# isabella232/Garfield

Hardware: AMD Instinct MI355X
Metric: img/sec ResNet-50 f=2 Multi-Krum (higher is better)
Workload: dtype bf16; 1 GPU; model=resnet50 (torchvision architecture, 10 classes, 23528522 params), global_batch=2000, parallelism=dp1 (robust DP, 8 logical workers/GPU, n=8), gar=krum, f=2, batch_per_worker=250, exchange_dtype=bf16, hip_graphs=True, worker_batching=True, lp_weights=True, optimizer=SGD lr=0.01 momentum=0.9 wd=5e-4 (fused into the GAR combine kernel)

## Files before the change

garfield_amd/csrc/bindings.cpp:

```cpp
#include <map>
#include <mutex>
#include <torch/extension.h>
#include <c10/hip/HIPGuard.h>
#include <c10/hip/HIPStream.h>

#include <cstdint>
#include <cstdlib>
#include <string>
#include <vector>

#include "bn_gpu.hpp"
#include "conv_f32.hpp"
#include "gar_common.hpp"
#include "gar_cpu.hpp"
#include "gar_gpu.hpp"
#include "loss_gpu.hpp"
#include "mailbox.hpp"
#include "threadpool.hpp"

namespace py = pybind11;
using garfield::RowTable;

namespace {

// ... 1399 lines not shown
  bool bf16 = false;
  int64_t ss = 0, gs = 0;
  if (out.scalar_type() == at::kFloat) {
    TORCH_CHECK(out.is_contiguous() && out.dim() == 4 && out.size(0) == splits && out.size(1) == groups &&
                    out.size(2) == cout && out.size(3) == K,
                "gpu_iwgrad: an fp32 out must be contiguous [splits, groups, Cout, K]");
    ss = groups * cout * K;
    gs = cout * K;
  } else {
    TORCH_CHECK(out.scalar_type() == at::kBFloat16 && splits == 1 && out.dim() == 3 && out.size(0) == groups &&
                    out.size(1) == cout && out.size(2) == K && out.stride(2) == 1 && out.stride(1) == K &&
                    out.stride(0) >= cout * K,
                "gpu_iwgrad: a bf16 out must be a [groups, Cout, K] view with contiguous rows (splits == 1)");
    bf16 = true;
    gs = out.stride(0);
  }
  const float* psc = opt_vec(pro_scale, groups * g.C, x.device(), "pro_scale");
  const float* psh = opt_vec(pro_shift, groups * g.C, x.device(), "pro_shift");
  TORCH_CHECK((psc == nullptr) == (psh == nullptr), "gpu_iwgrad: pass both pro_scale and pro_shift or neither");
  c10::hip::HIPGuard guard(x.device().index());
  if (psc) {
    TORCH_CHECK(kh == 1 && kw == 1 && sh == 1 && sw == 1 && ph == 0 && pw == 0,
                "gpu_iwgrad: the BatchNorm prologue takes 1x1 stride-1 unpadded convolutions only");
    garfield::gpu::iwgrad_nhwc(u16(x), u16(dy), g, static_cast<int>(cout), static_cast<int>(groups), M / groups,
                               static_cast<int>(splits), out.data_ptr(), bf16, ss, gs, stream_of(x.device()), psc, psh);
    return;
  }
  if (garfield::gpu::wgrad3x3_nhwc(u16(x), u16(dy), g, static_cast<int>(cout), static_cast<int>(groups),
                                         M / groups, static_cast<int>(splits), out.data_ptr(), bf16, ss, gs,
                                         stream_of(x.device())))
    return;
  garfield::gpu::iwgrad_nhwc(u16(x), u16(dy), g, static_cast<int>(cout), static_cast<int>(groups), M / groups,
                             static_cast<int>(splits), out.data_ptr(), bf16, ss, gs, stream_of(x.device()));
}

bool g_wgrad3x3_fits(int64_t n, int64_t h, int64_t w, int64_t c, int64_t cout, int64_t groups) {
  garfield::gpu::Im2col g{static_cast<int>(n), static_cast<int>(h), static_cast<int>(w), static_cast<int>(c), 3, 3,
                          1, 1, 1, 1, 1, 1, static_cast<int>(h), static_cast<int>(w), 0};
  if (groups < 1 || n % groups) return false;
  return garfield::gpu::wgrad3x3_fits(g, static_cast<int>(cout), n / groups * h * w);
}

garfield::gpu::Im2col pool_geometry(const at::Tensor& x, const at::Tensor& y, const at::Tensor& idx, int64_t k,
                                    int64_t s, int64_t p) {
  auto g = conv_geometry(x, k, k, s, s, p, p, 1, 1, true);
  TORCH_CHECK(g.C % 8 == 0 && reinterpret_cast<uintptr_t>(x.data_ptr()) % 16 == 0,
              "garfield maxpool: channels must be a multiple of 8 and x 16-byte aligned");
  TORCH_CHECK(y.device() == x.device() && y.scalar_type() == x.scalar_type() && y.dim() == 4 && y.size(0) == g.N &&
                  y.size(1) == g.C && y.size(2) == g.Ho && y.size(3) == g.Wo &&
                  y.is_contiguous(at::MemoryFormat::ChannelsLast) && reinterpret_cast<uintptr_t>(y.data_ptr()) % 16 == 0,
              "garfield maxpool: y must be a channels_last [", g.N, ", ", g.C, ", ", g.Ho, ", ", g.Wo, "] tensor of x's dtype");
  TORCH_CHECK(idx.device() == x.device() && idx.scalar_type() == at::kByte && idx.numel() == y.numel() &&
                  idx.is_contiguous() && reinterpret_cast<uintptr_t>(idx.data_ptr()) % 8 == 0 && k * k <= 256,
              "garfield maxpool: idx must be a contiguous uint8 tensor of y's element count");
  return g;
}

void g_maxpool_fwd(const at::Tensor& x, int64_t k, int64_t s, int64_t p, const at::Tensor& y, const at::Tensor& idx) {
  auto g = pool_geometry(x, y, idx, k, s, p);
  c10::hip::HIPGuard guard(x.device().index());
  garfield::gpu::maxpool_fwd_nhwc(x.data_ptr(), g, y.data_ptr(), static_cast<uint8_t*>(idx.data_ptr()),
                                  stream_of(x.device()), dtype_code(x));
}

void g_maxpool_bwd(const at::Tensor& dy, const at::Tensor& idx, int64_t k, int64_t s, int64_t p, const at::Tensor& dx) {
  auto g = pool_geometry(dx, dy, idx, k, s, p);
// ... 582 lines not shown
  m.def("gpu_iconv", &g_iconv, "Implicit-GEMM NHWC convolution on MFMA: y = conv(x, w) (+ add); args (x, w, kh, kw, "
        "sh, sw, ph, pw, dh, dw, y, add=None, pm=0, transpose_w=False); x/y/add channels_last bf16, C % 32 == 0, "
        "Cout % 64 == 0; transpose_w: w is the forward weight [C, Cout, KH, KW] whose flipped transpose is applied "
        "(the data gradient of that convolution); add_mask [y.numel() / 8] uint8: add counts where its bit is set "
        "(halo-staged 3x3 kernel only, y a separate tensor). Returns False when nothing was launched (add_mask on a "
        "shape the halo kernel does not take)",
        py::arg("x"), py::arg("w"), py::arg("kh"), py::arg("kw"), py::arg("sh"), py::arg("sw"), py::arg("ph"),
        py::arg("pw"), py::arg("dh"), py::arg("dw"), py::arg("y"), py::arg("add") = py::none(), py::arg("pm") = 0,
        py::arg("transpose_w") = false, py::arg("stats") = py::none(), py::arg("rg") = 0,
        py::arg("add_mask") = py::none());
  m.def("conv3x3_stats_rows", [](int64_t n, int64_t h, int64_t w, int64_t c, int64_t cout) -> int64_t {
          return 16 * g_conv3x3_pick(n, h, w, c, cout);
        }, py::arg("n"), py::arg("h"), py::arg("w"), py::arg("c"), py::arg("cout"),
        "Rows per statistics tile of the halo-staged 3x3 kernel's BatchNorm-statistics epilogue (0: no fit); "
        "the stats buffer holds ceil(M / rows) * 6 * Cout floats (E = 1)");

  m.def("gpu_sc_expand", &g_sc_expand, py::arg("weights"), py::arg("hs"), py::arg("ws"), py::arg("bigs"),
        py::arg("bigTs"), "Per-step expansion of 3x3 weights for images of at most 2x2 pixels: Wbig[(p', co), (p, ci)] "
        "= W[co, h - h' + 1, w - w' + 1, ci] (0 off the kernel) and its transpose, every layer in one launch");
  m.def("gpu_sc_fold", &g_sc_fold, py::arg("slab"), py::arg("h"), py::arg("w"), py::arg("out"),
        "Fold a dense small-image weight gradient (fp32 [S, G, P*Cout, P*Cin]) onto the nine taps: out[g, co, "
        "(i, j, ci)] = Σ_s Σ over the pixel pairs of tap (i, j)");
  m.def("gpu_dgrad_s2", &g_dgrad_s2, "Data gradient of a stride-2 convolution on MFMA without a dcol matrix: dx = "
        "conv_transpose(dy, w) (+ add, in place of add when given; dx may be add); args (dy, w, kh, kw, ph, pw, dx, "
        "add=None, pm=0); w the channels_last forward weight [C, Cout, KH, KW]", py::arg("dy"), py::arg("w"),
        py::arg("kh"), py::arg("kw"), py::arg("ph"), py::arg("pw"), py::arg("dx"), py::arg("add") = py::none(),
        py::arg("pm") = 0);
  m.def("dgrad_s2_ok", &g_dgrad_s2_ok, py::arg("dy"), py::arg("dx"), py::arg("kh"), py::arg("kw"), py::arg("ph"),
        py::arg("pw"), "True when gpu_dgrad_s2 takes this geometry");
  m.def("conv3x3_pick", &g_conv3x3_pick, py::arg("n"), py::arg("h"), py::arg("w"), py::arg("c"), py::arg("cout"),
        "Pixel fragments per wave the halo-staged 3x3 kernel uses for this NHWC shape (0: it does not fit)");
  m.def("wgrad3x3_fits", &g_wgrad3x3_fits, py::arg("n"), py::arg("h"), py::arg("w"), py::arg("c"), py::arg("cout"),
        py::arg("groups"), "True when gpu_iwgrad of this 3x3 / stride-1 / pad-1 shape runs the halo-staged kernel");
  m.def("gpu_iwgrad", &g_iwgrad, "Per-worker implicit-GEMM weight gradient on MFMA: out[s, g] = Σ over pixel "
        "split s of worker g of dyᵀ · patches(x); args (x, dy, kh, kw, sh, sw, ph, pw, dh, dw, groups, out, splits, "
        "pro_scale=None, pro_shift=None); pro_*: [groups, C] BatchNorm prologue of x (1x1 only)",
        py::arg("x"), py::arg("dy"), py::arg("kh"), py::arg("kw"), py::arg("sh"), py::arg("sw"), py::arg("ph"),
        py::arg("pw"), py::arg("dh"), py::arg("dw"), py::arg("groups"), py::arg("out"), py::arg("splits"),
        py::arg("pro_scale") = py::none(), py::arg("pro_shift") = py::none());
  m.def("gpu_conv_f32", &g_conv_f32, py::arg("src"), py::arg("w"), py::arg("kh"), py::arg("kw"),
        py::arg("sh"), py::arg("sw"), py::arg("ph"), py::arg("pw"), py::arg("dh"), py::arg("dw"), py::arg("dgrad"),
        py::arg("out"), py::arg("add") = py::none(), py::arg("pm") = 0, py::arg("ksplit") = 0,
        "fp32 NHWC implicit-GEMM convolution (forward, or with dgrad the data gradient of a convolution of this "
        "geometry, any stride) on split-bf16 MFMA (three bf16 pieces per operand, the six products of order <= 2, "
        "fp32 accumulation); w: the weight's pieces [3, Co, K]; pm 0: automatic kernel choice (split-K included "
        "unless ksplit is given), ksplit > 1: that many k-splits summed by a second pass");
  m.def("conv_f32_supported", [](int64_t cs, int64_t co) {
    garfield::gpu::ConvF32Geo g{};
    g.Cs = static_cast<int>(cs);
    g.Co = static_cast<int>(co);
    return garfield::gpu::conv_f32_supported(g);
  }, py::arg("cs"), py::arg("co"));
  m.def("gpu_wgrad_f32", &g_wgrad_f32, py::arg("x"), py::arg("dy"), py::arg("kh"), py::arg("kw"), py::arg("sh"),
        py::arg("sw"), py::arg("ph"), py::arg("pw"), py::arg("dh"), py::arg("dw"), py::arg("groups"), py::arg("out"),
        py::arg("splits"), py::arg("variant") = 0,
        "Per-worker fp32 weight gradient on split-bf16 MFMA (variant: 0 auto, 1 / 2 the 128x128 tile double- / "
        "single-buffered, 3 the 64x64 tile)");
  m.def("gpu_wsplit_multi", &g_wsplit_multi, "Per-step weight split of many fp32 weights: W -> its three bf16 "
        "pieces (row pitch ld) and, optionally, the channel-transposed pieces of the data gradient");
  m.def("gpu_linear_f32_fwd", [](const at::Tensor& x, const at::Tensor& w, const c10::optional<at::Tensor>& b,
                                 const at::Tensor& y) {
    const auto dev = x.device();
    const int64_t R = x.size(0), F = x.size(1), O = w.size(0);
    check_f32_mat(x, dev, R, F, "x");
    check_f32_mat(w, dev, O, F, "w");
    check_f32_mat(y, dev, R, O, "y");
// ... 315 lines not shown
```

garfield_amd/csrc/bn_gpu.hpp:

```cpp
#pragma once
#include <hip/hip_runtime.h>
#include <cstdint>

namespace garfield {
namespace gpu {

constexpr int kBnMaxChunks = 64;

int64_t bn_part_floats(int64_t rg, int groups, int C);

struct RunJob {
  const float* mean;
  const float* istd;
  float* run_mean;
  float* run_var;
  int64_t rg;
  int C;
  int groups;
  float eps;
  float momentum;
};
constexpr int kRunJobs = 48;
struct RunJobs {
  RunJob j[kRunJobs];
// ... 71 lines not shown
int conv3x3_pick(const Im2col& g, int Cout);
struct ScExpandJob {
  const uint16_t* w;
  uint16_t* big;
  uint16_t* bigT;
  int cout, cin, H, W;
};
constexpr int kScMaxJobs = 32;
struct ScExpandJobs {
  ScExpandJob job[kScMaxJobs];
  int64_t start[kScMaxJobs + 1];
  int count;
};
void sc_expand(const ScExpandJobs& jobs, hipStream_t stream);
void sc_fold(const float* slab, int S, int G, int H, int W, int cout, int cin, void* out, bool out_bf16,
             int64_t gstride, hipStream_t stream);

bool dgrad_s2_ok(const Im2col& g, int Cout);
void dgrad_s2_nhwc(const uint16_t* dy, const uint16_t* w, const Im2col& g, int Cout, uint16_t* dx, const uint16_t* add,
                   int pm, hipStream_t stream);
bool conv3x3_nhwc(const uint16_t* x, const uint16_t* w, const Im2col& g, int Cout, uint16_t* y, const uint16_t* add,
                  int pmf, hipStream_t stream, float* stats = nullptr, int64_t rg = 0,
                  const uint8_t* add_mask = nullptr);
bool wgrad3x3_fits(const Im2col& g, int Cout, int64_t rg);
bool wgrad3x3_nhwc(const uint16_t* x, const uint16_t* dy, const Im2col& g, int Cout, int groups, int64_t rg,
                   int splits, void* out, bool out_bf16, int64_t split_stride, int64_t group_stride,
                   hipStream_t stream);
void maxpool_fwd_nhwc(const void* x, const Im2col& g, void* y, uint8_t* idx, hipStream_t stream, int dt = 1);
void maxpool_bwd_nhwc(const void* dy, const uint8_t* idx, const Im2col& g, void* dx, hipStream_t stream, int dt = 1);
int iwgrad_taps_per_block(int kw, int kh = 3, int C = 0, int Cout = 0);
void iwgrad_nhwc(const uint16_t* x, const uint16_t* dy, const Im2col& g, int Cout, int groups, int64_t rg,
                 int splits, void* out, bool out_bf16, int64_t split_stride, int64_t group_stride, hipStream_t stream,
                 const float* pro_scale = nullptr, const float* pro_shift = nullptr);
void col2im_nhwc(const uint16_t* dcol, const Im2col& g, uint16_t* dx, bool accumulate, hipStream_t stream);

}
}
```

garfield_amd/csrc/iconv_nhwc.hip:

```cpp
#include <cstdlib>

#include "bn_gpu.hpp"
#include "gar_device.hpp"

namespace garfield {
namespace gpu {
using namespace dev;
namespace {

constexpr int kWaves = 4;

__device__ __forceinline__ bf16x8 pro_frag(bf16x8 b, float sc, float sh) {
  const uint4 u = __builtin_bit_cast(uint4, b);
  const float x[8] = {__uint_as_float(u.x << 16), __uint_as_float(u.x & 0xffff0000u),
                      __uint_as_float(u.y << 16), __uint_as_float(u.y & 0xffff0000u),
                      __uint_as_float(u.z << 16), __uint_as_float(u.z & 0xffff0000u),
                      __uint_as_float(u.w << 16), __uint_as_float(u.w & 0xffff0000u)};
  float y[8];
#pragma unroll
  for (int i = 0; i < 8; ++i) y[i] = fmaxf(fmaf(x[i], sc, sh), 0.f);
  return __builtin_bit_cast(bf16x8, make_uint4(pack_bf16x2(y[0], y[1]), pack_bf16x2(y[2], y[3]),
                                               pack_bf16x2(y[4], y[5]), pack_bf16x2(y[6], y[7])));
}

template <int PM>
struct Frags {
  bf16x8 a[4];
  bf16x8 b[PM];
};

template <int PM, bool ADD>
__global__ __launch_bounds__(256) void k_iconv(const uint16_t* __restrict__ x, const uint16_t* __restrict__ w,
                                               Im2col g, int Cout, uint16_t* y, const uint16_t* add) {
// ... 822 lines not shown
#pragma unroll
    for (int j = 0; j < NT; ++j)
#pragma unroll
      for (int v = 0; v < 2; ++v) {
        bf16x8 bx =
            __builtin_bit_cast(bf16x8, __builtin_shufflevector(rb[j][2 * v], rb[j][2 * v + 1], 0, 1, 2, 3, 4, 5, 6, 7));
        if constexpr (PRO) bx = pro_frag(bx, psv[j][v], phv[j][v]);
#pragma unroll
        for (int u = 0; u < 2; ++u)
          acc[j][u][v] = __builtin_amdgcn_mfma_f32_16x16x32_bf16(a[u], bx, acc[j][u][v], 0, 0, 0);
      }
  }

#pragma unroll
  for (int j = 0; j < NT; ++j) {
    const int k0 = c0 + j * 64;
#pragma unroll
    for (int u = 0; u < 2; ++u)
#pragma unroll
      for (int v = 0; v < 2; ++v)
#pragma unroll
        for (int e = 0; e < 4; ++e) {
          const int co = co0 + (cf0 + u) * 16 + 4 * grp + e;
          const int64_t o = static_cast<int64_t>(sp) * split_stride + static_cast<int64_t>(gi) * group_stride +
                            static_cast<int64_t>(co) * K + k0 + (kf0 + v) * 16 + li;
          if constexpr (OUT_BF16) static_cast<uint16_t*>(out)[o] = f_to_bf16(acc[j][u][v][e]);
          else static_cast<float*>(out)[o] = acc[j][u][v][e];
        }
  }
}

constexpr int kW1Stage = 4 * 64 * 128;

template <bool OUT_BF16, bool PRO, int NS = 3>
__global__ __launch_bounds__(256) void k_iwgrad_1x1_wide(const uint16_t* __restrict__ x, const uint16_t* __restrict__ dy,
                                                         Im2col g, int Cout, int64_t rg, int64_t per_split, void* out,
                                                         int64_t split_stride, int64_t group_stride,
                                                         const float* __restrict__ psc, const float* __restrict__ psh) {
  constexpr int SUB = 64 * 128;
  extern __shared__ __attribute__((aligned(16))) char wlds[];
  const int lane = threadIdx.x & 63, wave = threadIdx.x >> 6;
  const int K = g.C;
  const int nq = g.C / 128;
  const int qb = blockIdx.x % nq, cb = blockIdx.x / nq;
  const int c0 = qb * 128, co0 = cb * 128;
  const int gi = blockIdx.y, sp = blockIdx.z;
  const int64_t mbeg = static_cast<int64_t>(gi) * rg + static_cast<int64_t>(sp) * per_split;
  int64_t mend = mbeg + per_split;
  if (mend > static_cast<int64_t>(gi + 1) * rg) mend = static_cast<int64_t>(gi + 1) * rg;
  const int steps = mend > mbeg ? static_cast<int>((mend - mbeg + 63) / 64) : 0;
  const FastDiv fWo = make_fastdiv(g.Wo), fHo = make_fastdiv(g.Ho);
  const bool ident = g.sh == 1 && g.sw == 1 && g.ph == 0 && g.pw == 0 && g.H == g.Ho && g.W == g.Wo;

  const int lchunk = lane & 7;
  const uint16_t* zsrc = reinterpret_cast<const uint16_t*>(g_iconv_zero) + lchunk * 8;
  const uint64_t az = reinterpret_cast<uint64_t>(zsrc);
  auto issue = [&](int s, int slot) {
    char* base = wlds + slot * kW1Stage;
#pragma unroll
    for (int hb = 0; hb < 2; ++hb) {
      const int row = 8 * (hb * 4 + wave) + (lane >> 3);
      const int lsw = lchunk ^ (2 * tr_g(row));
      const int m = static_cast<int>(mbeg) + s * 64 + row;
      const bool mv = m < static_cast<int>(mend);
      const int mm = mv ? m : 0;
      bool ok = mv;
      int64_t xo = mm;
      if (!ident) {
        uint32_t t, wo, n, ho;
        fdivmod(static_cast<uint32_t>(mm), fWo, t, wo);
        fdivmod(t, fHo, n, ho);
        const int hi = static_cast<int>(ho) * g.sh - g.ph, wi = static_cast<int>(wo) * g.sw - g.pw;
        ok = mv && hi >= 0 && hi < g.H && wi >= 0 && wi < g.W;
        xo = (static_cast<int64_t>(n) * g.H + (ok ? hi : 0)) * g.W + (ok ? wi : 0);
      }
      const uint16_t* dr = dy + static_cast<int64_t>(mm) * Cout + co0 + lsw * 8;
      const uint16_t* xr = x + xo * g.C + c0 + lsw * 8;
#pragma unroll
      for (int b = 0; b < 2; ++b) {
// ... 52 lines not shown
          "ds_read_b64_tr_b16 %4, %18\n\t"
          "ds_read_b64_tr_b16 %5, %18 offset:512\n\t"
          "ds_read_b64_tr_b16 %6, %19\n\t"
          "ds_read_b64_tr_b16 %7, %19 offset:512\n\t"
          "ds_read_b64_tr_b16 %8, %20\n\t"
          "ds_read_b64_tr_b16 %9, %20 offset:512\n\t"
          "ds_read_b64_tr_b16 %10, %21\n\t"
          "ds_read_b64_tr_b16 %11, %21 offset:512\n\t"
          "ds_read_b64_tr_b16 %12, %22\n\t"
          "ds_read_b64_tr_b16 %13, %22 offset:512\n\t"
          "ds_read_b64_tr_b16 %14, %23\n\t"
          "ds_read_b64_tr_b16 %15, %23 offset:512\n\t"
          "s_waitcnt lgkmcnt(0)"
          : "=&v"(ra[0]), "=&v"(ra[1]), "=&v"(ra[2]), "=&v"(ra[3]), "=&v"(ra[4]), "=&v"(ra[5]), "=&v"(ra[6]),
            "=&v"(ra[7]), "=&v"(rb[0]), "=&v"(rb[1]), "=&v"(rb[2]), "=&v"(rb[3]), "=&v"(rb[4]), "=&v"(rb[5]),
            "=&v"(rb[6]), "=&v"(rb[7])
          : "v"(b0 + offA[0]), "v"(b0 + offA[1]), "v"(b0 + offA[2]), "v"(b0 + offA[3]), "v"(b0 + offB[0]),
            "v"(b0 + offB[1]), "v"(b0 + offB[2]), "v"(b0 + offB[3])
          : "memory");
      bf16x8 a[4], b[4];
#pragma unroll
      for (int k = 0; k < 4; ++k) {
        a[k] = __builtin_bit_cast(bf16x8, __builtin_shufflevector(ra[2 * k], ra[2 * k + 1], 0, 1, 2, 3, 4, 5, 6, 7));
        b[k] = __builtin_bit_cast(bf16x8, __builtin_shufflevector(rb[2 * k], rb[2 * k + 1], 0, 1, 2, 3, 4, 5, 6, 7));
        if constexpr (PRO) b[k] = pro_frag(b[k], psv[k], phv[k]);
      }
#pragma unroll
      for (int u = 0; u < 4; ++u)
#pragma unroll
        for (int v = 0; v < 4; ++v) acc[u][v] = __builtin_amdgcn_mfma_f32_16x16x32_bf16(a[u], b[v], acc[u][v], 0, 0, 0);
    }
  }

#pragma unroll
  for (int u = 0; u < 4; ++u)
#pragma unroll
    for (int v = 0; v < 4; ++v)
#pragma unroll
      for (int e = 0; e < 4; ++e) {
        const int co = co0 + (4 * sa + u) * 16 + 4 * grp + e;
        const int k = c0 + (4 * sbk + v) * 16 + li;
        const int64_t o = static_cast<int64_t>(sp) * split_stride + static_cast<int64_t>(gi) * group_stride +
                          static_cast<int64_t>(co) * K + k;
        if constexpr (OUT_BF16) static_cast<uint16_t*>(out)[o] = f_to_bf16(acc[u][v][e]);
        else static_cast<float*>(out)[o] = acc[u][v][e];
      }
}

int iwgrad_taps_per_block(int kw, int kh, int C, int Cout) {
  if (kw == 1 && kh == 1) return C % 128 == 0 ? (Cout % 128 == 0 ? 4 : 2) : 1;
  return kw == 3 ? 3 : 1;
}

template <bool PRO>
void iwgrad_launch(const uint16_t* x, const uint16_t* dy, const Im2col& g, int Cout, int groups, int64_t rg,
                   int splits, void* out, bool out_bf16, int64_t split_stride, int64_t group_stride, hipStream_t stream,
                   const float* psc, const float* psh) {
  const int K = g.KH * g.KW * g.C;
  if (splits < 1) splits = 1;
  const int64_t per_split = (rg + splits - 1) / splits;
  const int tpb = iwgrad_taps_per_block(g.KW, g.KH, g.C, Cout);
  if (tpb == 4 && g.KW == 1) {
    static bool once = (hipFuncSetAttribute(reinterpret_cast<const void*>(&k_iwgrad_1x1_wide<true, PRO>),
                                            hipFuncAttributeMaxDynamicSharedMemorySize, 3 * kW1Stage),
                        hipFuncSetAttribute(reinterpret_cast<const void*>(&k_iwgrad_1x1_wide<false, PRO>),
                                            hipFuncAttributeMaxDynamicSharedMemorySize, 3 * kW1Stage),
                        hipFuncSetAttribute(reinterpret_cast<const void*>(&k_iwgrad_1x1_wide<true, PRO, 2>),
                                            hipFuncAttributeMaxDynamicSharedMemorySize, 2 * kW1Stage),
                        hipFuncSetAttribute(reinterpret_cast<const void*>(&k_iwgrad_1x1_wide<false, PRO, 2>),
                                            hipFuncAttributeMaxDynamicSharedMemorySize, 2 * kW1Stage),
                        true);
    (void)once;
    const dim3 grid((g.C / 128) * (Cout / 128), groups, splits);
    const bool ns2 = (per_split + 63) / 64 <= 4;
    if (out_bf16 && ns2)
      hipLaunchKernelGGL((k_iwgrad_1x1_wide<true, PRO, 2>), grid, dim3(256), 2 * kW1Stage, stream, x, dy, g, Cout, rg,
                         per_split, out, split_stride, group_stride, psc, psh);
    else if (out_bf16)
      hipLaunchKernelGGL((k_iwgrad_1x1_wide<true, PRO>), grid, dim3(256), 3 * kW1Stage, stream, x, dy, g, Cout, rg,
// ... 7 lines not shown
    return;
  }
  if (tpb == 2 && g.KW == 1) {
    const dim3 grid((g.C / 128) * (Cout / 64), groups, splits);
    if (out_bf16)
      hipLaunchKernelGGL((k_iwgrad_1x1<3, true, 2, PRO>), grid, dim3(256), 0, stream, x, dy, g, Cout, rg, per_split,
                         out, split_stride, group_stride, psc, psh);
    else
      hipLaunchKernelGGL((k_iwgrad_1x1<3, false, 2, PRO>), grid, dim3(256), 0, stream, x, dy, g, Cout, rg, per_split,
                         out, split_stride, group_stride, psc, psh);
    return;
  }
  if constexpr (!PRO) {
    if (tpb == 3) {
      const dim3 grid(g.KH * (g.C / 64) * (Cout / 64), groups, splits);
      if (out_bf16)
        hipLaunchKernelGGL((k_iwgrad_rows<3, true, 1>), grid, dim3(256), 0, stream, x, dy, g, Cout, rg, per_split, out,
                           split_stride, group_stride);
      else
        hipLaunchKernelGGL((k_iwgrad_rows<3, false, 1>), grid, dim3(256), 0, stream, x, dy, g, Cout, rg, per_split, out,
                           split_stride, group_stride);
      return;
    }
  }
  const dim3 grid((K / 64) * (Cout / 64), groups, splits);
  if (out_bf16)
    hipLaunchKernelGGL((k_iwgrad<3, true, PRO>), grid, dim3(256), 0, stream, x, dy, g, Cout, rg, per_split, out,
                       split_stride, group_stride, psc, psh);
  else
    hipLaunchKernelGGL((k_iwgrad<3, false, PRO>), grid, dim3(256), 0, stream, x, dy, g, Cout, rg, per_split, out,
                       split_stride, group_stride, psc, psh);
}

void iwgrad_nhwc(const uint16_t* x, const uint16_t* dy, const Im2col& g, int Cout, int groups, int64_t rg,
                 int splits, void* out, bool out_bf16, int64_t split_stride, int64_t group_stride, hipStream_t stream,
                 const float* pro_scale, const float* pro_shift) {
  if (pro_scale)
    iwgrad_launch<true>(x, dy, g, Cout, groups, rg, splits, out, out_bf16, split_stride, group_stride, stream,
                        pro_scale, pro_shift);
  else
    iwgrad_launch<false>(x, dy, g, Cout, groups, rg, splits, out, out_bf16, split_stride, group_stride, stream, nullptr,
                         nullptr);
}

}
}
```

garfield_amd/ops/grouped.py:

```python
from __future__ import annotations

import math

import torch
import torch.nn.functional as F

from garfield_amd import _native
from garfield_amd.ops import tuning
from garfield_amd.utils.flat import is_dense

ICONV = True
IWGRAD = True
IWGRAD_1X1 = True
STEM = True
_STEM_WG = 1024
XENT = True
GEMM_NT = True
GEMM_NT_DGRAD = True
CONV3X3 = True
BN_PROLOGUE = False
S2_DGRAD = True
_S2_CHOICE: dict = tuning.register("s2", {})
S2_FORCE = False
SMALL_CONV = True
LAZY_RES = True
FOLD_SHORTCUT_BN = True
BN_DUAL = True


def rows2d(t: torch.Tensor) -> torch.Tensor:
    if t.dim() == 2:
        return t
    if not t.is_contiguous(memory_format=torch.channels_last):
        raise ValueError("grouped layers need channels_last activations")
    return t.permute(0, 2, 3, 1).reshape(-1, t.shape[1])


def from_rows(t2: torch.Tensor, n: int, h: int, w: int) -> torch.Tensor:
    return t2.view(n, h, w, t2.shape[1]).permute(0, 3, 1, 2)


def _cl(t: torch.Tensor) -> torch.Tensor:
    return t.contiguous(memory_format=torch.channels_last) if t.dim() == 4 else t.contiguous()




class GradSink:

    def __init__(self, flat: torch.Tensor, row_stride: int, base: int, offsets: dict, groups: int):
        self.flat = flat
        self.row_stride = int(row_stride)
        self.base = int(base)
        self.offsets = offsets
        self.groups = int(groups)
        self._srcs: list = []
        self._offs: list = []
        self._split_parts: list = []
        self._split_outs: list = []
        self.defer_splits = True

    def offset(self, p: torch.Tensor) -> int:
        return self.offsets[id(p)]

    def row_offset(self, g: int, p: torch.Tensor) -> int:
        return self.base + g * self.row_stride + self.offsets[id(p)]

    def put(self, p: torch.Tensor, g: int, grad: torch.Tensor) -> None:
        if grad.numel() != p.numel():
            raise ValueError(f"gradient of {grad.numel()} elements for a parameter of {p.numel()}")
        self._srcs.append(grad)
        self._offs.append(self.row_offset(g, p))

    def rows_view(self, p: torch.Tensor, shape: tuple, dtype: torch.dtype) -> torch.Tensor | None:
        if self.flat.dtype != dtype:
            return None
        strides, acc = [], 1
        for d in reversed(shape):
            strides.append(acc)
            acc *= int(d)
        if acc != p.numel():
            raise ValueError(f"rows_view of {acc} elements for a parameter of {p.numel()}")
        return self.flat.as_strided((self.groups, *shape), (self.row_stride, *reversed(strides)),
                                    self.base + self.offsets[id(p)])

    def queue_split(self, part: torch.Tensor, out: torch.Tensor) -> None:
        if self.defer_splits and part.is_cuda:
            self._split_parts.append(part)
            self._split_outs.append(out)
        else:
            _native.native().gpu_split_reduce(part, out)

    def put_groups(self, p: torch.Tensor, grads) -> None:
        for g in range(self.groups):
            self.put(p, g, grads[g])

    def flush_splits(self) -> None:
        if self._split_parts:
            _native.native().gpu_split_reduce_multi(self._split_parts, self._split_outs)
            self._split_parts.clear()
            self._split_outs.clear()

    def flush(self) -> None:
        self.flush_splits()
        if not self._srcs:
            return
        if self.flat.is_cuda:
            srcs = [s if is_dense(s) else s.contiguous() for s in self._srcs]
            _native.native().gpu_flatten_cast_at(srcs, self._offs, self.flat)
        else:
            with torch.no_grad():
                for s, o in zip(self._srcs, self._offs):
                    v = _memory_order(s)
                    self.flat[o:o + v.numel()].copy_(v)
        self._srcs.clear()
        self._offs.clear()


def _memory_order(t: torch.Tensor) -> torch.Tensor:
    if t.is_contiguous():
        return t.reshape(-1)
    perm = sorted(range(t.dim()), key=lambda i: -t.stride(i))
    return t.permute(perm).reshape(-1)


class GradJoin:

    __slots__ = ("pending", "lazy")

    def __init__(self):
# ... 253 lines not shown
        else:
            dx2, dr2 = _bn_bwd_ref(x2, dy2, y2, st, ctx.has_res)
            dx = from_rows(dx2, n, h, w)
            dres = from_rows(dr2, n, h, w) if dr2 is not None else None
        if lazy is not None:
            if ctx.join is not None:
                ctx.join.park(lazy)
            else:
                ctx.res_link.pending = lazy
        elif dres is not None and ctx.join is not None:
            ctx.join.park(dres)
            dres = None
        return dx, None, None, dres, None, None, None, None, None, None


def grouped_bn(x, st: BNState, ws: Workspace, res=None, res_join: GradJoin | None = None,
               res_link: ResLink | None = None, out_link: ResLink | None = None, res_st: BNState | None = None):
    return _GroupedBN.apply(_cl(x), st.bn.weight, st.bn.bias, _cl(res) if res is not None else None, st, ws,
                            res_join, res_link, out_link, res_st)




class ConvSpec:
    def __init__(self, conv: torch.nn.Conv2d, sink: GradSink | None, groups: int):
        if conv.groups != 1 or conv.bias is not None:
            raise ValueError("grouped convolution supports groups=1 convolutions without bias")
        self.conv = conv
        self.sink = sink
        self.groups = groups
        self.kernel = tuple(conv.kernel_size)
        self.stride = tuple(conv.stride)
        self.padding = tuple(conv.padding)
        self.dilation = tuple(conv.dilation)
        self.gemm = (self.kernel == (1, 1) and self.stride == (1, 1) and self.padding == (0, 0)
                     and self.dilation == (1, 1))
        self.bn_next = None
        self.wpad = None
        self.wt = None
        self.dcol = False
        self.wd = None
        self.flip = False
        self.w3 = self.wt3 = None
        self.sc = None
        self.wbig = self.wbigT = None


def _gemm_nt_ok(a2: torch.Tensor, b2: torch.Tensor) -> bool:
    M, K = a2.shape
    N = b2.shape[0]
    return (a2.is_cuda and a2.dtype == torch.bfloat16 and b2.dtype == torch.bfloat16 and K % 64 == 0
            and N % 64 == 0 and b2.shape[1] == K and a2.is_contiguous() and b2.is_contiguous()
            and M * max(K, N) < 2 ** 31)


_GEMM_CFG: dict = tuning.register("gemm", {})


def _gemm_cfg(a2: torch.Tensor, b2: torch.Tensor, rg: int, add: torch.Tensor | None, pro=None) -> int:
    C_ = _native.native()
    M, K = a2.shape
    N = b2.shape[0]
    key = (M, N, K, rg, add is not None, pro is not None)
    cfg = _GEMM_CFG.get(key)
    if cfg is not None:
        return cfg
# ... 377 lines not shown
    while S < _IWGRAD_MAXS and tiles * S < _IWGRAD_WG and rows_per_worker // (2 * S) >= _IWGRAD_MINPIX:
        S *= 2
    return S


def _wgrad3x3_splits(rows_per_worker: int, blocks: int) -> int:
    tiles = -(-rows_per_worker // 128)
    S = 1
    while S < 64 and blocks * S < _WGRAD3_WG and tiles // (2 * S) >= _WGRAD3_MINTILES:
        S *= 2
    return S


_WGRAD3_WG = 512
_WGRAD3_MINTILES = 3


_IWGRAD_WG = 512
_IWGRAD_MINPIX = 512
_IWGRAD_MAXS = 64


def _iwgrad(x: torch.Tensor, dy: torch.Tensor, spec: "ConvSpec", G: int, K: int, pro=None) -> None:
    pkw = {} if pro is None else {"pro_scale": pro[0], "pro_shift": pro[1]}
    cout = dy.shape[1]
    rows = dy.shape[0] * dy.shape[2] * dy.shape[3] // G
    C_ = _native.native()
    if (CONV3X3 and spec.kernel == (3, 3) and spec.stride == (1, 1) and spec.padding == (1, 1)
            and spec.dilation == (1, 1) and C_.wgrad3x3_fits(x.shape[0], x.shape[2], x.shape[3], x.shape[1], cout, G)):
        S = _wgrad3x3_splits(rows, (x.shape[1] // 64) * (cout // 64) * G)
    else:
        S = _iwgrad_splits(rows, (K // 64) * (cout // 64) * G //
                          C_.iwgrad_taps_per_block(spec.kernel[1], spec.kernel[0], x.shape[1], cout))
    out = spec.sink.rows_view(spec.conv.weight, (cout, K), dy.dtype) if S == 1 else None
    if out is not None:
        C_.gpu_iwgrad(x, dy, *_geom(spec), G, out, 1, **pkw)
        return
    part = torch.empty((S, G, cout, K), dtype=torch.float32, device=dy.device)
    C_.gpu_iwgrad(x, dy, *_geom(spec), G, part, S, **pkw)
    rows = spec.sink.rows_view(spec.conv.weight, (cout, K), spec.sink.flat.dtype)
    if rows is not None:
        spec.sink.queue_split(part, rows)
    else:
        spec.sink.put_groups(spec.conv.weight, part.sum(0) if S > 1 else part[0])


def _stem_kind(w: torch.Tensor, spec: "ConvSpec") -> int | None:
    if spec.dilation != (1, 1):
        return None
    if tuple(w.shape) == (64, 3, 7, 7) and spec.stride == (2, 2) and spec.padding == (3, 3):
        return 0
    if tuple(w.shape) == (64, 3, 3, 3) and spec.stride == (1, 1) and spec.padding == (1, 1):
        return 1
    return None


def _stem_ok(x: torch.Tensor, w: torch.Tensor, spec: "ConvSpec") -> bool:
    kind = _stem_kind(w, spec)
    return (STEM and kind is not None and x.is_cuda and x.dtype == torch.bfloat16 and w.dtype == torch.bfloat16
            and _channels_last_weight(w) and x.is_contiguous(memory_format=torch.channels_last)
            and _native.native().stem_supported(x.shape[2], x.shape[3], kind))


def _stem_wgrad(x: torch.Tensor, dy: torch.Tensor, spec: "ConvSpec", G: int) -> None:
    per = x.shape[0] // G
    wg = _STEM_WG * (2 if dy.shape[2] * dy.shape[3] > 4096 else 1)
    S = max(1, min(per, -(-wg // G)))
    C_ = _native.native()
    kind = _stem_kind(spec.conv.weight, spec) or 0
    K = C_.stem_k(kind)
    part = torch.empty((S, G, 64, K), dtype=torch.float32, device=dy.device)
    C_.gpu_stem_wgrad(x, dy, G, part, kind)
    rows = spec.sink.rows_view(spec.conv.weight, (64, K), spec.sink.flat.dtype)
# ... 787 lines not shown
```

garfield_amd/parallel/grouped.py:

```python
from __future__ import annotations

import torch
import torch.nn as nn
import torch.nn.functional as F

from garfield_amd.models.resnet import BasicBlock, Bottleneck, ResNet
from garfield_amd.parallel.signals import DeviceSignal
from garfield_amd.ops.grouped import (BNState, ConvSpec, GradJoin, GradSink, LinearSpec, ResLink, Workspace,
                                      bn_conv_ok, global_avgpool, grouped_bn, grouped_bn_conv, grouped_conv,
                                      grouped_cross_entropy, grouped_linear, grouped_maxpool, refresh_dgrad_weights,
                                      refresh_f32_weights, refresh_sc_weights)
import garfield_amd.ops.grouped as _gops


def supports(model: nn.Module) -> bool:
    if not isinstance(model, ResNet):
        return False
    for m in model.modules():
        if isinstance(m, nn.BatchNorm2d):
            if m.num_features % 8 or m.momentum is None or not m.affine:
                return False
        elif isinstance(m, nn.Conv2d):
            if m.groups != 1 or m.bias is not None:
                return False
# ... 22 lines not shown
            kh, kw = mod.kernel_size
            if mod is not model.conv1 and kh * kw > 1 and tuple(mod.stride) != (1, 1):
                sizes.append(out.numel() // mod.out_channels * mod.in_channels * kh * kw)

    hooks = [m.register_forward_hook(hook) for m in model.modules()
             if isinstance(m, (nn.Conv2d, nn.BatchNorm2d, nn.MaxPool2d, nn.ReLU, nn.Linear, nn.AdaptiveAvgPool2d))]
    state = {n: torch.empty_like(t, device="meta") for n, t in [*model.named_parameters(), *model.named_buffers()]}
    try:
        with torch.no_grad():
            torch.func.functional_call(model, state, (torch.empty((rows, *sample_shape), device="meta"),))
    finally:
        for h in hooks:
            h.remove()
    _CAPACITY[key] = out = max(sizes)
    return out


def fits(model: ResNet, rows: int, sample_shape) -> bool:
    return largest_index(model, rows, sample_shape) <= INDEX_LIMIT


class GroupedResNet:

    def __init__(self, model: ResNet, groups: int, sink: GradSink, loss_fn=F.cross_entropy, marks=(),
                 offsets: dict | None = None, signals: bool = True):
        if not supports(model):
            raise ValueError("GroupedResNet supports the zoo's ResNet models only")
        self.model = model
        self.groups = int(groups)
        self.sink = sink
        self.loss_fn = loss_fn
        self.ws = Workspace()
        self.conv = {m: ConvSpec(m, sink, self.groups) for m in model.modules() if isinstance(m, nn.Conv2d)}
        self.fc = LinearSpec(model.fc, sink, self.groups)
        self.bn: dict = {}
        self._seed = None
        self.join_residuals = True
        self.marks = tuple(marks)
        self._offsets = offsets or {}
        self._events = None
        self._end = None
        if signals and self.marks and next(model.parameters()).is_cuda:
            dev = next(model.parameters()).device
            self._events = {name: DeviceSignal(dev) for name in self.marks}
            self._end = DeviceSignal(dev)

    def bucket_offsets(self) -> list:
        out = []
        for name in self.marks:
            layer = getattr(self.model, name)
            offs = [self._offsets[id(p)] for p in layer.parameters() if id(p) in self._offsets]
            if offs:
                out.append(min(offs))
        return out

    def mark_events(self):
        if self._events is None:
            return None
        return [self._events[name] for name in self.marks] + [self._end]

    def replayed(self) -> None:
        for sgn in self.mark_events() or ():
            sgn.replayed()


    def _state(self, bn: nn.BatchNorm2d, relu: bool) -> BNState:
# ... 155 lines not shown
```

Measured before the change: 380,000 img/s.

## Batch small 1x1 weight-gradient GEMMs into one multi-job kernel launch per stage

Adds a multi-job variant of the wide 1x1 weight-gradient kernel that takes up to 16 layer jobs in one grid, with blocks mapped to jobs through prefix offsets and jobs sorted by work. Small 1x1 wgrad calls (fewer than 512 workgroups, no BN prologue) are queued in the gradient sink and flushed per ResNet stage or before split reduction. The aim is to cut launch count and fill the GPU better when individual layers launch too few workgroups. It delays wgrad work and keeps activations alive until the flush, and it adds a per-block linear job search.

After: 388,600 img/s, median of 6. 1.02x the previous value.

```diff
diff --git a/garfield_amd/csrc/bindings.cpp b/garfield_amd/csrc/bindings.cpp
--- a/garfield_amd/csrc/bindings.cpp
+++ b/garfield_amd/csrc/bindings.cpp
@@ -1455,6 +1455,69 @@
     return;
   garfield::gpu::iwgrad_nhwc(u16(x), u16(dy), g, static_cast<int>(cout), static_cast<int>(groups), M / groups,
                              static_cast<int>(splits), out.data_ptr(), bf16, ss, gs, stream_of(x.device()));
+}
+
+void g_iwgrad_multi(const std::vector<at::Tensor>& xs, const std::vector<at::Tensor>& dys,
+                    const std::vector<std::vector<int64_t>>& geoms, int64_t groups, const std::vector<at::Tensor>& outs,
+                    const std::vector<int64_t>& splits) {
+  const size_t n = xs.size();
+  TORCH_CHECK(dys.size() == n && geoms.size() == n && outs.size() == n && splits.size() == n,
+              "gpu_iwgrad_multi: xs, dys, geoms, outs and splits must have one entry per job");
+  if (n == 0) return;
+  std::vector<garfield::gpu::WgJob> jobs;
+  jobs.reserve(n);
+  const at::Device dev = xs[0].device();
+  int64_t wgs = 0;
+  for (size_t i = 0; i < n; ++i) {
+    const at::Tensor &x = xs[i], &dy = dys[i], &out = outs[i];
+    const auto& q = geoms[i];
+    TORCH_CHECK(q.size() == 8, "gpu_iwgrad_multi: a geometry is (kh, kw, sh, sw, ph, pw, dh, dw)");
+    TORCH_CHECK(x.device() == dev, "gpu_iwgrad_multi: every job must be on one device");
+    auto g = conv_geometry(x, q[0], q[1], q[2], q[3], q[4], q[5], q[6], q[7]);
+    TORCH_CHECK(dy.is_cuda() && dy.device() == dev && dy.scalar_type() == at::kBFloat16 && dy.dim() == 4 &&
+                    dy.is_contiguous(at::MemoryFormat::ChannelsLast) && dy.size(0) == g.N && dy.size(2) == g.Ho &&
+                    dy.size(3) == g.Wo,
+                "gpu_iwgrad_multi: dy must be a channels_last bf16 [", g.N, ", Cout, ", g.Ho, ", ", g.Wo, "] tensor");
+    const int64_t cout = dy.size(1);
+    TORCH_CHECK(cout <= INT32_MAX && garfield::gpu::iwgrad_wide_ok(g, static_cast<int>(cout)),
+                "gpu_iwgrad_multi: takes 1x1 convolutions with input and output channels multiples of 128 only (got ",
+                g.KH, "x", g.KW, ", ", g.C, " -> ", cout, ")");
+    const int64_t M = static_cast<int64_t>(g.N) * g.Ho * g.Wo;
+    TORCH_CHECK(groups >= 1 && M % groups == 0, "gpu_iwgrad_multi: ", M, " output pixels do not split into ", groups,
+                " workers");
+    TORCH_CHECK(M < INT32_MAX && static_cast<int64_t>(g.N) * g.H * g.W * g.C < INT32_MAX,
+                "gpu_iwgrad_multi: tensor too large");
+    const int64_t S = splits[i];
+    TORCH_CHECK(S >= 1 && S <= 64, "gpu_iwgrad_multi: splits must be in [1, 64]");
+    TORCH_CHECK(reinterpret_cast<uintptr_t>(x.data_ptr()) % 16 == 0 && reinterpret_cast<uintptr_t>(dy.data_ptr()) % 16 == 0,
+                "gpu_iwgrad_multi: x and dy must be 16-byte aligned");
+    const int64_t K = g.C;
+    TORCH_CHECK(out.device() == dev, "gpu_iwgrad_multi: out must be on x's device");
+    bool bf16 = false;
+    int64_t ss = 0, gs = 0;
+    if (out.scalar_type() == at::kFloat) {
+      TORCH_CHECK(out.is_contiguous() && out.dim() == 4 && out.size(0) == S && out.size(1) == groups &&
+                      out.size(2) == cout && out.size(3) == K,
+                  "gpu_iwgrad_multi: an fp32 out must be contiguous [splits, groups, Cout, K]");
+      ss = groups * cout * K;
+      gs = cout * K;
+    } else {
+      TORCH_CHECK(out.scalar_type() == at::kBFloat16 && S == 1 && out.dim() == 3 && out.size(0) == groups &&
+                      out.size(1) == cout && out.size(2) == K && out.stride(2) == 1 && out.stride(1) == K &&
+                      out.stride(0) >= cout * K,
+                  "gpu_iwgrad_multi: a bf16 out must be a [groups, Cout, K] view with contiguous rows (splits == 1)");
+      bf16 = true;
+      gs = out.stride(0);
+    }
+    const int64_t rg = M / groups;
+    wgs += (g.C / 128) * (cout / 128) * groups * S;
+    TORCH_CHECK(wgs < INT32_MAX, "gpu_iwgrad_multi: too many workgroups");
+    jobs.push_back(garfield::gpu::WgJob{u16(x), u16(dy), out.data_ptr(), rg, (rg + S - 1) / S, ss, gs, g,
+                                       static_cast<int>(cout), static_cast<int>(groups), static_cast<int>(S),
+                                       bf16 ? 1 : 0});
+  }
+  c10::hip::HIPGuard guard(dev.index());
+  garfield::gpu::iwgrad_wide_multi(jobs.data(), static_cast<int>(jobs.size()), stream_of(dev));
 }
 
 bool g_wgrad3x3_fits(int64_t n, int64_t h, int64_t w, int64_t c, int64_t cout, int64_t groups) {
@@ -2103,6 +2166,10 @@
         "Pixel fragments per wave the halo-staged 3x3 kernel uses for this NHWC shape (0: it does not fit)");
   m.def("wgrad3x3_fits", &g_wgrad3x3_fits, py::arg("n"), py::arg("h"), py::arg("w"), py::arg("c"), py::arg("cout"),
         py::arg("groups"), "True when gpu_iwgrad of this 3x3 / stride-1 / pad-1 shape runs the halo-staged kernel");
+  m.def("gpu_iwgrad_multi", &g_iwgrad_multi, py::arg("xs"), py::arg("dys"), py::arg("geoms"), py::arg("groups"),
+        py::arg("outs"), py::arg("splits"),
+        "gpu_iwgrad of several 1x1 layers (input and output channels multiples of 128, no prologue) in one "
+        "launch per 16 jobs; every job's result is bitwise what gpu_iwgrad writes for it");
   m.def("gpu_iwgrad", &g_iwgrad, "Per-worker implicit-GEMM weight gradient on MFMA: out[s, g] = Σ over pixel "
         "split s of worker g of dyᵀ · patches(x); args (x, dy, kh, kw, sh, sw, ph, pw, dh, dw, groups, out, splits, "
         "pro_scale=None, pro_shift=None); pro_*: [groups, C] BatchNorm prologue of x (1x1 only)",
diff --git a/garfield_amd/csrc/bn_gpu.hpp b/garfield_amd/csrc/bn_gpu.hpp
--- a/garfield_amd/csrc/bn_gpu.hpp
+++ b/garfield_amd/csrc/bn_gpu.hpp
@@ -127,6 +127,23 @@
 void iwgrad_nhwc(const uint16_t* x, const uint16_t* dy, const Im2col& g, int Cout, int groups, int64_t rg,
                  int splits, void* out, bool out_bf16, int64_t split_stride, int64_t group_stride, hipStream_t stream,
                  const float* pro_scale = nullptr, const float* pro_shift = nullptr);
+struct WgJob {
+  const uint16_t* x;
+  const uint16_t* dy;
+  void* out;
+  int64_t rg, per_split, split_stride, group_stride;
+  Im2col g;
+  int Cout, groups, splits;
+  int out_bf16;
+};
+constexpr int kWgJobs = 16;
+struct WgJobs {
+  WgJob j[kWgJobs];
+  int start[kWgJobs];
+  int n;
+};
+bool iwgrad_wide_ok(const Im2col& g, int Cout);
+void iwgrad_wide_multi(const WgJob* jobs, int count, hipStream_t stream);
 void col2im_nhwc(const uint16_t* dcol, const Im2col& g, uint16_t* dx, bool accumulate, hipStream_t stream);
 
 }
diff --git a/garfield_amd/csrc/iconv_nhwc.hip b/garfield_amd/csrc/iconv_nhwc.hip
--- a/garfield_amd/csrc/iconv_nhwc.hip
+++ b/garfield_amd/csrc/iconv_nhwc.hip
@@ -1,4 +1,6 @@
+#include <algorithm>
 #include <cstdlib>
+#include <type_traits>
 
 #include "bn_gpu.hpp"
 #include "gar_device.hpp"
@@ -887,19 +889,19 @@
 
 constexpr int kW1Stage = 4 * 64 * 128;
 
-template <bool OUT_BF16, bool PRO, int NS = 3>
-__global__ __launch_bounds__(256) void k_iwgrad_1x1_wide(const uint16_t* __restrict__ x, const uint16_t* __restrict__ dy,
-                                                         Im2col g, int Cout, int64_t rg, int64_t per_split, void* out,
-                                                         int64_t split_stride, int64_t group_stride,
-                                                         const float* __restrict__ psc, const float* __restrict__ psh) {
+template <bool PRO, int NS>
+__device__ __forceinline__ void iwgrad_wide_body(const uint16_t* __restrict__ x, const uint16_t* __restrict__ dy,
+                                                 const Im2col& g, int Cout, int64_t rg, int64_t per_split, void* out,
+                                                 bool out_bf16, int64_t split_stride, int64_t group_stride,
+                                                 const float* __restrict__ psc, const float* __restrict__ psh,
+                                                 int tile, int gi, int sp) {
   constexpr int SUB = 64 * 128;
   extern __shared__ __attribute__((aligned(16))) char wlds[];
   const int lane = threadIdx.x & 63, wave = threadIdx.x >> 6;
   const int K = g.C;
   const int nq = g.C / 128;
-  const int qb = blockIdx.x % nq, cb = blockIdx.x / nq;
+  const int qb = tile % nq, cb = tile / nq;
   const int c0 = qb * 128, co0 = cb * 128;
-  const int gi = blockIdx.y, sp = blockIdx.z;
   const int64_t mbeg = static_cast<int64_t>(gi) * rg + static_cast<int64_t>(sp) * per_split;
   int64_t mend = mbeg + per_split;
   if (mend > static_cast<int64_t>(gi + 1) * rg) mend = static_cast<int64_t>(gi + 1) * rg;
@@ -1018,19 +1020,47 @@
     }
   }
 
-#pragma unroll
-  for (int u = 0; u < 4; ++u)
-#pragma unroll
-    for (int v = 0; v < 4; ++v)
-#pragma unroll
-      for (int e = 0; e < 4; ++e) {
-        const int co = co0 + (4 * sa + u) * 16 + 4 * grp + e;
-        const int k = c0 + (4 * sbk + v) * 16 + li;
-        const int64_t o = static_cast<int64_t>(sp) * split_stride + static_cast<int64_t>(gi) * group_stride +
-                          static_cast<int64_t>(co) * K + k;
-        if constexpr (OUT_BF16) static_cast<uint16_t*>(out)[o] = f_to_bf16(acc[u][v][e]);
-        else static_cast<float*>(out)[o] = acc[u][v][e];
-      }
+  auto store = [&](auto bf) {
+#pragma unroll
+    for (int u = 0; u < 4; ++u)
+#pragma unroll
+      for (int v = 0; v < 4; ++v)
+#pragma unroll
+        for (int e = 0; e < 4; ++e) {
+          const int co = co0 + (4 * sa + u) * 16 + 4 * grp + e;
+          const int k = c0 + (4 * sbk + v) * 16 + li;
+          const int64_t o = static_cast<int64_t>(sp) * split_stride + static_cast<int64_t>(gi) * group_stride +
+                            static_cast<int64_t>(co) * K + k;
+          if constexpr (decltype(bf)::value) static_cast<uint16_t*>(out)[o] = f_to_bf16(acc[u][v][e]);
+          else static_cast<float*>(out)[o] = acc[u][v][e];
+        }
+  };
+  if (out_bf16) store(std::true_type{});
+  else store(std::false_type{});
+}
+
+template <bool OUT_BF16, bool PRO, int NS = 3>
+__global__ __launch_bounds__(256) void k_iwgrad_1x1_wide(const uint16_t* __restrict__ x, const uint16_t* __restrict__ dy,
+                                                         Im2col g, int Cout, int64_t rg, int64_t per_split, void* out,
+                                                         int64_t split_stride, int64_t group_stride,
+                                                         const float* __restrict__ psc, const float* __restrict__ psh) {
+  iwgrad_wide_body<PRO, NS>(x, dy, g, Cout, rg, per_split, out, OUT_BF16, split_stride, group_stride, psc, psh,
+                            static_cast<int>(blockIdx.x), static_cast<int>(blockIdx.y), static_cast<int>(blockIdx.z));
+}
+
+template <int NS>
+__global__ __launch_bounds__(256) void k_iwgrad_1x1_wide_multi(WgJobs jobs) {
+  const int bid = static_cast<int>(blockIdx.x);
+  int j = 0;
+  for (int i = 1; i < jobs.n; ++i)
+    if (bid >= jobs.start[i]) j = i;
+  const WgJob& jb = jobs.j[j];
+  const int tiles = (jb.g.C / 128) * (jb.Cout / 128);
+  const int r = bid - jobs.start[j];
+  const int tile = r % tiles, t = r / tiles;
+  const int gi = t % jb.groups, sp = t / jb.groups;
+  iwgrad_wide_body<false, NS>(jb.x, jb.dy, jb.g, jb.Cout, jb.rg, jb.per_split, jb.out, jb.out_bf16 != 0,
+                              jb.split_stride, jb.group_stride, nullptr, nullptr, tile, gi, sp);
 }
 
 int iwgrad_taps_per_block(int kw, int kh, int C, int Cout) {
@@ -1104,6 +1134,43 @@
                        split_stride, group_stride, psc, psh);
 }
 
+bool iwgrad_wide_ok(const Im2col& g, int Cout) {
+  return g.KH == 1 && g.KW == 1 && g.C % 128 == 0 && Cout % 128 == 0;
+}
+
+void iwgrad_wide_multi(const WgJob* jobs, int count, hipStream_t stream) {
+  static bool once = (hipFuncSetAttribute(reinterpret_cast<const void*>(&k_iwgrad_1x1_wide_multi<3>),
+                                          hipFuncAttributeMaxDynamicSharedMemorySize, 3 * kW1Stage),
+                      hipFuncSetAttribute(reinterpret_cast<const void*>(&k_iwgrad_1x1_wide_multi<2>),
+                                          hipFuncAttributeMaxDynamicSharedMemorySize, 2 * kW1Stage),
+                      true);
+  (void)once;
+  for (int b = 0; b < count; b += kWgJobs) {
+    const int n = count - b < kWgJobs ? count - b : kWgJobs;
+    int order[kWgJobs];
+    int64_t steps[kWgJobs];
+    for (int i = 0; i < n; ++i) {
+      order[i] = i;
+      steps[i] = (jobs[b + i].per_split + 63) / 64;
+    }
+    std::stable_sort(order, order + n, [&](int a, int c) { return steps[a] > steps[c]; });
+    WgJobs wj{};
+    int64_t total = 0;
+    bool ns2 = true;
+    for (int i = 0; i < n; ++i) {
+      const WgJob& jb = jobs[b + order[i]];
+      wj.j[i] = jb;
+      wj.start[i] = static_cast<int>(total);
+      total += static_cast<int64_t>(jb.g.C / 128) * (jb.Cout / 128) * jb.groups * jb.splits;
+      ns2 = ns2 && steps[order[i]] <= 4;
+    }
+    wj.n = n;
+    const dim3 grid(static_cast<unsigned>(total));
+    if (ns2) hipLaunchKernelGGL(k_iwgrad_1x1_wide_multi<2>, grid, dim3(256), 2 * kW1Stage, stream, wj);
+    else hipLaunchKernelGGL(k_iwgrad_1x1_wide_multi<3>, grid, dim3(256), 3 * kW1Stage, stream, wj);
+  }
+}
+
 void iwgrad_nhwc(const uint16_t* x, const uint16_t* dy, const Im2col& g, int Cout, int groups, int64_t rg,
                  int splits, void* out, bool out_bf16, int64_t split_stride, int64_t group_stride, hipStream_t stream,
                  const float* pro_scale, const float* pro_shift) {
diff --git a/garfield_amd/ops/grouped.py b/garfield_amd/ops/grouped.py
--- a/garfield_amd/ops/grouped.py
+++ b/garfield_amd/ops/grouped.py
@@ -26,6 +26,9 @@
 LAZY_RES = True
 FOLD_SHORTCUT_BN = True
 BN_DUAL = True
+WGRAD_BATCH = True
+_WGRAD_BATCH_MAXWG = 2 * 256
+_WGRAD_BATCH_FLUSH_WG = 0
 
 
 def rows2d(t: torch.Tensor) -> torch.Tensor:
@@ -59,6 +62,9 @@
         self._split_parts: list = []
         self._split_outs: list = []
         self.defer_splits = True
+        self._wq: list = []
+        self._wq_wgs = 0
+        self._wq_stage = None
 
     def offset(self, p: torch.Tensor) -> int:
         return self.offsets[id(p)]
@@ -95,7 +101,25 @@
         for g in range(self.groups):
             self.put(p, g, grads[g])
 
+    def queue_wgrad(self, x: torch.Tensor, dy: torch.Tensor, geom: tuple, out: torch.Tensor, splits: int,
+                    wgs: int, stage=None) -> None:
+        if self._wq and not _WGRAD_BATCH_FLUSH_WG and stage != self._wq_stage:
+            self.flush_wgrads()
+        self._wq_stage = stage
+        self._wq.append((x, dy, list(geom), out, splits))
+        self._wq_wgs += wgs
+        if _WGRAD_BATCH_FLUSH_WG and self._wq_wgs >= _WGRAD_BATCH_FLUSH_WG:
+            self.flush_wgrads()
+
+    def flush_wgrads(self) -> None:
+        if self._wq:
+            xs, dys, geoms, outs, splits = (list(c) for c in zip(*self._wq))
+            self._wq.clear()
+            self._wq_wgs = 0
+            _native.native().gpu_iwgrad_multi(xs, dys, geoms, self.groups, outs, splits)
+
     def flush_splits(self) -> None:
+        self.flush_wgrads()
         if self._split_parts:
             _native.native().gpu_split_reduce_multi(self._split_parts, self._split_outs)
             self._split_parts.clear()
@@ -415,6 +439,7 @@
         self.kernel = tuple(conv.kernel_size)
         self.stride = tuple(conv.stride)
         self.padding = tuple(conv.padding)
+        self.stage = None
         self.dilation = tuple(conv.dilation)
         self.gemm = (self.kernel == (1, 1) and self.stride == (1, 1) and self.padding == (0, 0)
                      and self.dilation == (1, 1))
@@ -858,13 +883,22 @@
     else:
         S = _iwgrad_splits(rows, (K // 64) * (cout // 64) * G //
                           C_.iwgrad_taps_per_block(spec.kernel[1], spec.kernel[0], x.shape[1], cout))
+    wgs = (K // 128) * (cout // 128) * G * S
+    batch = (WGRAD_BATCH and pro is None and spec.kernel == (1, 1) and K % 128 == 0 and cout % 128 == 0
+             and wgs < _WGRAD_BATCH_MAXWG and isinstance(spec.sink, GradSink) and spec.sink.groups == G)
     out = spec.sink.rows_view(spec.conv.weight, (cout, K), dy.dtype) if S == 1 else None
     if out is not None:
-        C_.gpu_iwgrad(x, dy, *_geom(spec), G, out, 1, **pkw)
+        if batch:
+            spec.sink.queue_wgrad(x, dy, _geom(spec), out, 1, wgs, spec.stage)
+        else:
+            C_.gpu_iwgrad(x, dy, *_geom(spec), G, out, 1, **pkw)
         return
     part = torch.empty((S, G, cout, K), dtype=torch.float32, device=dy.device)
-    C_.gpu_iwgrad(x, dy, *_geom(spec), G, part, S, **pkw)
     rows = spec.sink.rows_view(spec.conv.weight, (cout, K), spec.sink.flat.dtype)
+    if batch and rows is not None and spec.sink.defer_splits:
+        spec.sink.queue_wgrad(x, dy, _geom(spec), part, S, wgs, spec.stage)
+    else:
+        C_.gpu_iwgrad(x, dy, *_geom(spec), G, part, S, **pkw)
     if rows is not None:
         spec.sink.queue_split(part, rows)
     else:
diff --git a/garfield_amd/parallel/grouped.py b/garfield_amd/parallel/grouped.py
--- a/garfield_amd/parallel/grouped.py
+++ b/garfield_amd/parallel/grouped.py
@@ -78,6 +78,10 @@
         self.loss_fn = loss_fn
         self.ws = Workspace()
         self.conv = {m: ConvSpec(m, sink, self.groups) for m in model.modules() if isinstance(m, nn.Conv2d)}
+        for name in ("layer1", "layer2", "layer3", "layer4"):
+            for c in getattr(model, name).modules():
+                if isinstance(c, nn.Conv2d):
+                    self.conv[c].stage = name
         self.fc = LinearSpec(model.fc, sink, self.groups)
         self.bn: dict = {}
         self._seed = None
```
